# InternetMaximalism/plonky2_bn254

Hardware: NVIDIA B200
Metric: g1_scalar_mul_stark_proofs_per_sec (higher is better)
Workload: dtype u64

## Files before the change

### plonky2_bn254_b200/csrc/merkle.cuh

```cuda
#pragma once
#include "poseidon.cuh"
#include "poseidon_tc.cuh"

namespace merkle {

using poseidon::Digest;

struct LeafHashK {
  const u64* lde;
  size_t stride;
  int W, log_n;
  Digest* out;
  int natural = 0;
  PB_HD void operator()(size_t j) const {
    u64 s[12];
#pragma unroll
    for (int i = 0; i < 12; i++) s[i] = 0;
    if (W <= 4) {
      for (int c = 0; c < W; c++) s[c] = lde[(size_t)c * stride + j];
    } else {
      int c = 0;
      for (; c + 8 <= W; c += 8) {
#pragma unroll
        for (int k = 0; k < 8; k++) s[k] = lde[(size_t)(c + k) * stride + j];
        poseidon::permute(s);
      }
      if (c < W) {
        for (int k = 0; c + k < W; k++) s[k] = lde[(size_t)(c + k) * stride + j];
        poseidon::permute(s);
      }
    }
    Digest d;
#pragma unroll
    for (int i = 0; i < 4; i++) d.e[i] = s[i];
    out[natural ? j : (size_t)gl::brev32((u32)j, log_n)] = d;
  }
};

struct RowHashK {
  const u64* rows;
  int len;
  Digest* out;
  PB_HD void operator()(size_t i) const {
    u64 s[12];
#pragma unroll
    for (int k = 0; k < 12; k++) s[k] = 0;
    const u64* row = rows + i * (size_t)len;
    if (len <= 4) {
      for (int c = 0; c < len; c++) s[c] = row[c];
    } else {
      for (int c = 0; c < len; c += 8) {
        for (int k = 0; k < 8 && c + k < len; k++) s[k] = row[c + k];
        poseidon::permute(s);
      }
    }
    Digest d;
#pragma unroll
    for (int k = 0; k < 4; k++) d.e[k] = s[k];
    out[i] = d;
  }
};

struct LevelK {
  const Digest* child;
  Digest* parent;
  PB_HD void operator()(size_t i) const { parent[i] = poseidon::two_to_one(child[2 * i], child[2 * i + 1]); }
};

#if !PB_HOSTSIM
__device__ __forceinline__ void stage_rc2(u64* rc2) {
  for (int i = threadIdx.x; i < poseidon::RC2_WORDS; i += blockDim.x) rc2[i] = poseidon::RC2_DEV[i];
  __syncthreads();
}

__global__ void __launch_bounds__(poseidon::tc::CTA, poseidon::tc::CTAS_PER_SM)
    k_leaf_hash_tc(const u64* __restrict__ lde, size_t stride, int W, int log_n, Digest* __restrict__ out, size_t rows,
                   int natural) {
  extern __shared__ unsigned char tc_dyn[];
  __shared__ u64 tc_bar;
  __shared__ u32 tc_slot[2];
  poseidon::tc::Ctx ctx;
  poseidon::tc::setup(ctx, tc_dyn, &tc_bar, tc_slot);
  const size_t j = (size_t)blockIdx.x * blockDim.x + threadIdx.x;
  const bool live = j < rows;
  const u64* p = lde + (live ? j : 0);
  u64 s[12];
#pragma unroll
  for (int i = 0; i < 12; i++) s[i] = 0;
  const int chunks = (W + 7) / 8;
#pragma unroll 1
  for (int c = 0; c < chunks; c++) {
    const int len = W - 8 * c;
    const u64* q = p + (size_t)c * 8 * stride;
#pragma unroll
    for (int k = 0; k < 8; k++)
      if (k < len) s[k] = q[(size_t)k * stride];
    poseidon::tc::permute(s, ctx);
  }
  if (live) {
    Digest d;
#pragma unroll
    for (int i = 0; i < 4; i++) d.e[i] = s[i];
    out[natural ? j : (size_t)gl::brev32((u32)j, log_n)] = d;
  }
  poseidon::tc::teardown(ctx);
}

__global__ void __launch_bounds__(128, 6) k_level(const Digest* __restrict__ child, Digest* __restrict__ parent, size_t n) {
  __shared__ __align__(16) u64 rc2[poseidon::RC2_WORDS];
  stage_rc2(rc2);
  const size_t i = (size_t)blockIdx.x * blockDim.x + threadIdx.x;
  if (i >= n) return;
  u64 s[12];
  const Digest l = child[2 * i], r = child[2 * i + 1];
#pragma unroll
  for (int k = 0; k < 4; k++) {
    s[k] = l.e[k];
    s[4 + k] = r.e[k];
    s[8 + k] = 0;
  }
  poseidon::lazy::permute(s, rc2);
  Digest d;
#pragma unroll
  for (int k = 0; k < 4; k++) d.e[k] = s[k];
  parent[i] = d;
}
#endif

static inline size_t tree_digests(int log_n, int cap_height) {
  size_t total = 0;
  for (int l = log_n; l >= cap_height; l--) total += (size_t)1 << l;
  return total;
}
static inline size_t level_offset(int log_n, int lvl) {
  size_t off = 0;
  for (int l = 0; l < lvl; l++) off += (size_t)1 << (log_n - l);
  return off;
}

static inline void launch_level(const Digest* child, Digest* parent, size_t n, pbStream s) {
#if PB_HOSTSIM
  LevelK k{child, parent};
  pb_launch("merkle level", k, n, s, 128);
#else
  k_level<<<(unsigned)((n + 127) / 128), 128, 0, s>>>(child, parent, n);
  g_pb_launches++;
  pb_check_last("merkle level");
#endif
}
static inline void build_levels(Digest* digests, int log_n, int cap_height, pbStream s) {
  if (cap_height > log_n) throw Pb254Error(6, "merkle: cap_height > log2(leaves)");
  size_t off = 0;
  for (int l = 0; l < log_n - cap_height; l++) {
    size_t m = (size_t)1 << (log_n - l);
    launch_level(digests + off, digests + off + m, m / 2, s);
    off += m;
  }
}

static inline void build_from_lde(const u64* lde, size_t stride, int W, int log_n, int cap_height, Digest* digests,
                                  pbStream s) {
#if PB_HOSTSIM
  LeafHashK k{lde, stride, W, log_n, digests};
  pb_launch("leaf hash", k, (size_t)1 << log_n, s, 128);
#else
  if (W <= 4) {
    LeafHashK k{lde, stride, W, log_n, digests};
    pb_launch("leaf copy", k, (size_t)1 << log_n, s, 128);
  } else {
    const size_t n = (size_t)1 << log_n;
    k_leaf_hash_tc<<<(unsigned)((n + 127) / 128), poseidon::tc::CTA, poseidon::tc::SMEM_BYTES, s>>>(lde, stride, W, log_n,
                                                                                                  digests, n, 0);
    g_pb_launches++;
    pb_check_last("leaf hash");
  }
#endif
  build_levels(digests, log_n, cap_height, s);
}
static inline void build_from_rows(const u64* rows, int len, int log_n, int cap_height, Digest* digests, pbStream s) {
  RowHashK k{rows, len, digests};
  pb_launch("row hash", k, (size_t)1 << log_n, s, 128);
  build_levels(digests, log_n, cap_height, s);
}


static inline void hash_rows_natural(const u64* m, size_t stride, int W, size_t rows, Digest* out, pbStream s) {
#if PB_HOSTSIM
  LeafHashK k{m, stride, W, 0, out, 1};
  pb_launch("leaf hash (rows)", k, rows, s, 128);
#else
  if (W <= 4) {
    LeafHashK k{m, stride, W, 0, out, 1};
    pb_launch("leaf copy (rows)", k, rows, s, 128);
  } else {
    k_leaf_hash_tc<<<(unsigned)((rows + 127) / 128), poseidon::tc::CTA, poseidon::tc::SMEM_BYTES, s>>>(m, stride, W, 0, out,
                                                                                                     rows, 1);
    g_pb_launches++;
    pb_check_last("leaf hash (rows)");
  }
#endif
}
struct SubtreeLeavesK {
  const Digest* all;
  Digest* leaves;
  size_t first;
  int log_N;
  PB_HD void operator()(size_t q) const { leaves[q] = all[gl::brev32((u32)(first + q), log_N)]; }
};

}
```

### plonky2_bn254_b200/csrc/poseidon_tc.cuh

```cuda
#pragma once
#include "poseidon.cuh"

#if !PB_HOSTSIM
namespace poseidon {
namespace tc {

static constexpr int CTA = 128;
static constexpr int A_BYTES = 128 * 128;
static constexpr int B_BYTES = 96 * 128;
static constexpr int CTAS_PER_SM = 5;
static constexpr int SMEM_BYTES = 41 * 1024;
static_assert(A_BYTES + 2 * B_BYTES + 1024 <= SMEM_BYTES && SMEM_BYTES <= 48 * 1024, "shared-memory plan");
__host__ __device__ constexpr u32 idesc(u32 n) { return (2u << 4) | ((n >> 3) << 17) | ((128u >> 4) << 24); }

static __device__ const uint4 B_IMAGE[B_BYTES / 16] = {
#include "poseidon_constants_tcb.inc"
};
static __device__ const uint4 BF_IMAGE[B_BYTES / 16] = {
#include "poseidon_constants_tcf.inc"
};

__device__ __forceinline__ u32 smem_u32(const void* p) { return (u32)__cvta_generic_to_shared(p); }

__device__ __forceinline__ u64 smem_desc(u32 addr) {
  return (u64)((addr & 0x3FFFFu) >> 4) | ((u64)(1024u >> 4) << 32) | (1ull << 46) | (2ull << 61);
}

struct Ctx {
  unsigned char* row;
  u32 r7;
  u32 bar;
  u32 tmem0, tmem1;
  u64 adesc, bdesc, bfdesc;
  u32 parity;
};

__device__ __forceinline__ void setup(Ctx& c, unsigned char* dyn, u64* bar, u32* slot) {
  const u32 t = threadIdx.x;
  unsigned char* base = dyn + ((1024u - (smem_u32(dyn) & 1023u)) & 1023u);
  unsigned char* a = base;
  unsigned char* b = base + A_BYTES;
  unsigned char* bf = b + B_BYTES;
  for (int i = t; i < B_BYTES / 16; i += CTA) {
    reinterpret_cast<uint4*>(b)[i] = B_IMAGE[i];
    reinterpret_cast<uint4*>(bf)[i] = BF_IMAGE[i];
  }
  c.row = a + t * 128;
  c.r7 = t & 7;
  c.bar = smem_u32(bar);
  if (t == 0) {
    asm volatile("mbarrier.init.shared::cta.b64 [%0], 1;" ::"r"(c.bar));
    asm volatile("fence.mbarrier_init.release.cluster;" ::: "memory");
  }
  if (t < 32) {
    asm volatile("tcgen05.alloc.cta_group::1.sync.aligned.shared::cta.b32 [%0], 64;" ::"r"(smem_u32(slot)) : "memory");
    asm volatile("tcgen05.alloc.cta_group::1.sync.aligned.shared::cta.b32 [%0], 32;" ::"r"(smem_u32(slot + 1)) : "memory");
    asm volatile("tcgen05.relinquish_alloc_permit.cta_group::1.sync.aligned;" ::: "memory");
  }
  asm volatile("tcgen05.fence::before_thread_sync;" ::: "memory");
  __syncthreads();
  asm volatile("tcgen05.fence::after_thread_sync;" ::: "memory");
  c.tmem0 = reinterpret_cast<volatile u32*>(slot)[0];
  c.tmem1 = reinterpret_cast<volatile u32*>(slot)[1];
  c.adesc = smem_desc(smem_u32(a));
  c.bdesc = smem_desc(smem_u32(b));
  c.bfdesc = smem_desc(smem_u32(bf));
  c.parity = 0;
}

__device__ __forceinline__ void teardown(const Ctx& c) {
  asm volatile("tcgen05.fence::before_thread_sync;" ::: "memory");
  __syncthreads();
  if (threadIdx.x < 32) {
    asm volatile("tcgen05.dealloc.cta_group::1.sync.aligned.b32 %0, 64;" ::"r"(c.tmem0) : "memory");
    asm volatile("tcgen05.dealloc.cta_group::1.sync.aligned.b32 %0, 32;" ::"r"(c.tmem1) : "memory");
  }
}

template <u32 N>
__device__ __forceinline__ void mma_i8(u32 d_tmem, u64 adesc, u64 bdesc, u32 accumulate) {
  asm volatile(
      "{\n\t"
      ".reg .pred p;\n\t"
      "setp.ne.b32 p, %4, 0;\n\t"
      "tcgen05.mma.cta_group::1.kind::i8 [%0], %1, %2, %3, p;\n\t"
      "}" ::"r"(d_tmem),
      "l"(adesc), "l"(bdesc), "n"(idesc(N)), "r"(accumulate)
      : "memory");
}

#define PB_TMEM_LD32(v, addr)                                                                                       \
  asm volatile(                                                                                                     \
      "tcgen05.ld.sync.aligned.32x32b.x32.b32 {%0, %1, %2, %3, %4, %5, %6, %7, %8, %9, %10, %11, %12, %13, %14, "   \
      "%15, %16, %17, %18, %19, %20, %21, %22, %23, %24, %25, %26, %27, %28, %29, %30, %31}, [%32];"                \
      : "=r"(v[0]), "=r"(v[1]), "=r"(v[2]), "=r"(v[3]), "=r"(v[4]), "=r"(v[5]), "=r"(v[6]), "=r"(v[7]), "=r"(v[8]), \
        "=r"(v[9]), "=r"(v[10]), "=r"(v[11]), "=r"(v[12]), "=r"(v[13]), "=r"(v[14]), "=r"(v[15]), "=r"(v[16]),      \
        "=r"(v[17]), "=r"(v[18]), "=r"(v[19]), "=r"(v[20]), "=r"(v[21]), "=r"(v[22]), "=r"(v[23]), "=r"(v[24]),     \
        "=r"(v[25]), "=r"(v[26]), "=r"(v[27]), "=r"(v[28]), "=r"(v[29]), "=r"(v[30]), "=r"(v[31])                   \
      : "r"(addr)                                                                                                   \
      : "memory")

__device__ __forceinline__ u64 recombine4(u32 acc0, u32 acc1, u32 acc2, u32 acc3) {
  const u32 t1 = __byte_perm(acc1, 0, 0x1044), u1 = __byte_perm(acc1, 0, 0x4432);
  const u32 t3 = __byte_perm(acc3, 0, 0x1044), u3 = __byte_perm(acc3, 0, 0x4432);
  u32 lo, hi;
  asm("{\n\t"
      ".reg .u32 w2, c;\n\t"
      "add.cc.u32   %0, %2, %3;\n\t"
      "addc.u32     %1, %4, %5;\n\t"
      "add.cc.u32   %1, %1, %6;\n\t"
      "addc.u32     w2, %7, 0;\n\t"
      "add.cc.u32   %1, %1, w2;\n\t"
      "addc.u32     c, 0, 0;\n\t"
      "sub.cc.u32   %0, %0, w2;\n\t"
      "subc.u32     %1, %1, 0;\n\t"
      "sub.u32      c, 0, c;\n\t"
      "add.cc.u32   %0, %0, c;\n\t"
      "addc.u32     %1, %1, 0;\n\t"
      "}"
      : "=&r"(lo), "=&r"(hi)
      : "r"(acc0), "r"(t1), "r"(u1), "r"(acc2), "r"(t3), "r"(u3));
  return ((u64)hi << 32) | lo;
}

__device__ __forceinline__ u64 fold8(const u32* q) {
  return recombine4(q[0] + (q[1] << 8), q[2] + (q[3] << 8), q[4] + (q[5] << 8), q[6] + (q[7] << 8));
}


__device__ __forceinline__ u32 onehot(int p, int w) { return (p >> 2) == w ? 1u << ((p & 3) * 8) : 0u; }

__device__ __forceinline__ u32 complement4(const u64 s[12], int i0, int i1, int i2, int i3) {
  const u32 a = __byte_perm((u32)(s[i0] >> 32), (u32)(s[i1] >> 32), 0x0073);
  const u32 b = __byte_perm((u32)(s[i2] >> 32), (u32)(s[i3] >> 32), 0x0073);
  return ~__byte_perm(a, b, 0x5410);
}

__device__ __forceinline__ void product(u64 s[12], Ctx& c, u64 bdesc, uint4 x6, uint4 x7) {
#pragma unroll
  for (int ch = 0; ch < 6; ch++)
    *reinterpret_cast<uint4*>(c.row + ((ch ^ c.r7) << 4)) =
        make_uint4((u32)s[2 * ch], (u32)(s[2 * ch] >> 32), (u32)s[2 * ch + 1], (u32)(s[2 * ch + 1] >> 32));
  *reinterpret_cast<uint4*>(c.row + ((6 ^ c.r7) << 4)) = x6;
  *reinterpret_cast<uint4*>(c.row + ((7 ^ c.r7) << 4)) = x7;
  asm volatile("fence.proxy.async.shared::cta;" ::: "memory");
  asm volatile("tcgen05.fence::before_thread_sync;" ::: "memory");
  __syncthreads();
  if (threadIdx.x == 0) {
    asm volatile("tcgen05.fence::after_thread_sync;" ::: "memory");
#pragma unroll
    for (int k = 0; k < 4; k++) {
      mma_i8<64>(c.tmem0, c.adesc + 2 * k, bdesc + 2 * k, k > 0);
      mma_i8<32>(c.tmem1, c.adesc + 2 * k, bdesc + (64 * 128 >> 4) + 2 * k, k > 0);
    }
    asm volatile("tcgen05.commit.cta_group::1.mbarrier::arrive::one.shared::cluster.b64 [%0];" ::"r"(c.bar) : "memory");
  }
  {
    u32 ok;
    do {
      asm volatile(
          "{\n\t"
          ".reg .pred p;\n\t"
          "mbarrier.try_wait.parity.shared::cta.b64 p, [%1], %2;\n\t"
          "selp.u32 %0, 1, 0, p;\n\t"
          "}"
          : "=r"(ok)
          : "r"(c.bar), "r"(c.parity)
          : "memory");
    } while (!ok);
    c.parity ^= 1;
  }
  asm volatile("tcgen05.fence::after_thread_sync;" ::: "memory");
  {
    const u32 lane_off = ((threadIdx.x >> 5) * 32u) << 16;
    const u32 t0 = c.tmem0 + lane_off, t1 = c.tmem0 + lane_off + 32, t2 = c.tmem1 + lane_off;
#define PB_TC_FOLD(a, base)                                                                                   \
  _Pragma("unroll") for (int r = 0; r < 4; r++) {                                                             \
    const u32* q = a + 8 * r;                                                                                 \
    s[base + r] = fold8(q);                                                                                   \
  }
    u32 a[32], b[32];
    PB_TMEM_LD32(a, t0);
    asm volatile("tcgen05.wait::ld.sync.aligned;" ::: "memory");
    PB_TMEM_LD32(b, t1);
    PB_TC_FOLD(a, 0)
    asm volatile("tcgen05.wait::ld.sync.aligned;" ::: "memory");
    PB_TMEM_LD32(a, t2);
    PB_TC_FOLD(b, 4)
    asm volatile("tcgen05.wait::ld.sync.aligned;" ::: "memory");
    PB_TC_FOLD(a, 8)
#undef PB_TC_FOLD
  }
}

__device__ __forceinline__ void permute(u64 s[12], Ctx& c) {
#pragma unroll
  for (int i = 0; i < 12; i++) {
    const u64 k = RC_DEV[i];
    u64 t = s[i] + k;
    if (t < k) t += gl::EPS;
    s[i] = t;
  }
  constexpr int N_FUSED = N_PARTIAL / 2, N_LAYERS = 2 * HALF_FULL + N_FUSED;
#pragma unroll 1
  for (int L = 0; L < N_LAYERS; L++) {
    uint4 x6, x7;
    u64 bdesc;
    if (L < HALF_FULL || L >= HALF_FULL + N_FUSED) {
#pragma unroll 1
      for (int j = 0; j < 2; j++) {
        u64 t[6];
#pragma unroll
        for (int i = 0; i < 6; i++) t[i] = lazy::sbox(s[i]);
#pragma unroll
        for (int i = 0; i < 6; i++) {
          s[i] = s[i + 6];
          s[i + 6] = t[i];
        }
      }
      const int R = L < HALF_FULL ? L : L + N_FUSED;
      const int p = R < N_ROUNDS - 1 ? R : -1;
      x6 = make_uint4(onehot(p, 0), onehot(p, 1), onehot(p, 2), onehot(p, 3));
      x7 = make_uint4(onehot(p, 4), onehot(p, 5), onehot(p, 6), onehot(p, 7));
      bdesc = c.bdesc;
    } else {
      const int j = L - HALF_FULL, r = HALF_FULL + 2 * j;
      s[0] = lazy::sbox(s[0]);
      u32 X[6][4];
#pragma unroll
      for (int k = 0; k < 6; k++) {
        const u32 a0 = (u32)s[2 * k], a1 = (u32)(s[2 * k] >> 32), b0 = (u32)s[2 * k + 1], b1 = (u32)(s[2 * k + 1] >> 32);
        X[k][0] = __byte_perm(a0, b0, 0x5410);
        X[k][1] = __byte_perm(a0, b0, 0x7632);
        X[k][2] = __byte_perm(a1, b1, 0x5410);
        X[k][3] = __byte_perm(a1, b1, 0x7632);
      }
      const uint4 k0 = *reinterpret_cast<const uint4*>(RC2_DEV + (r + 1) * 24);
      u32 acc[4] = {k0.x, k0.y, k0.z, k0.w};
      lazy::dp_row<0, 0>(acc, X);
      const u64 t = lazy::sbox(recombine4(acc[0], acc[1], acc[2], acc[3]));
      const int p = 8 + j;
      x6 = make_uint4((u32)t, (u32)(t >> 32), onehot(p, 2), onehot(p, 3));
      x7 = make_uint4(onehot(p, 4) | (~(u32)(s[0] >> 32) & 0xFF000000u), complement4(s, 1, 2, 3, 4),
                      complement4(s, 5, 6, 7, 8), complement4(s, 9, 10, 11, 11) & 0x00FFFFFFu);
      bdesc = c.bfdesc;
    }
    product(s, c, bdesc, x6, x7);
  }
#pragma unroll
  for (int i = 0; i < 12; i++) s[i] = s[i] >= gl::P ? s[i] - gl::P : s[i];
}

}
}
#endif
```

Baseline: 5.184.

## Overlap Poseidon TC operand staging with sbox and add L2 prefetch in leaf hash

Leaf hashing moves into a grid-strided tile loop and issues L2 prefetches for the next column chunk or tile while the current permutation runs. In the fused partial rounds, the shared-memory operand rows are written early and the s[0] sbox is split out of the dot-product. Its contribution is added afterwards with dp2a, so independent work can interleave with the sbox latency. Probe template hooks are added but compile to no-ops; the grid size is unchanged, so the tile loop runs once per block.

Measured after the change: 5.199 (median of 6 runs). About the same (+0.3%).

```diff
diff --git a/plonky2_bn254_b200/csrc/merkle.cuh b/plonky2_bn254_b200/csrc/merkle.cuh
--- a/plonky2_bn254_b200/csrc/merkle.cuh
+++ b/plonky2_bn254_b200/csrc/merkle.cuh
@@ -73,6 +73,53 @@
   __syncthreads();
 }
 
+__device__ __forceinline__ void prefetch_next_chunk(const u64* lde, size_t stride, int W, size_t rows, size_t tile,
+                                                    int c) {
+  const u32 t = threadIdx.x;
+  const int col = 8 * c + (int)(t >> 3);
+  const size_t row = tile * poseidon::tc::CTA + 16 * (t & 7);
+  if (t < 64 && col < W && row < rows)
+    asm volatile("prefetch.global.L2 [%0];" ::"l"(lde + (size_t)col * stride + row));
+}
+
+template <class Probe>
+__device__ __forceinline__ void leaf_hash_tiles(poseidon::tc::Ctx& ctx, const u64* __restrict__ lde, size_t stride,
+                                                int W, int log_n, Digest* __restrict__ out, size_t rows, int natural,
+                                                Probe& pr) {
+  const size_t tiles = (rows + poseidon::tc::CTA - 1) / poseidon::tc::CTA;
+  const int chunks = (W + 7) / 8;
+#pragma unroll 1
+  for (size_t tile = blockIdx.x; tile < tiles; tile += gridDim.x) {
+    pr.tile(tile);
+    const size_t j = tile * poseidon::tc::CTA + threadIdx.x;
+    const bool live = j < rows;
+    const u64* p = lde + (live ? j : 0);
+    u64 s[12];
+#pragma unroll
+    for (int i = 0; i < 12; i++) s[i] = 0;
+#pragma unroll 1
+    for (int c = 0; c < chunks; c++) {
+      const int len = W - 8 * c;
+      const u64* q = p + (size_t)c * 8 * stride;
+#pragma unroll
+      for (int k = 0; k < 8; k++)
+        if (k < len) s[k] = q[(size_t)k * stride];
+      prefetch_next_chunk(lde, stride, W, rows, c + 1 < chunks ? tile : tile + gridDim.x, c + 1 < chunks ? c + 1 : 0);
+      poseidon::tc::permute(s, ctx, pr);
+    }
+    if (live) {
+      Digest d;
+#pragma unroll
+      for (int i = 0; i < 4; i++) d.e[i] = s[i];
+      out[natural ? j : (size_t)gl::brev32((u32)j, log_n)] = d;
+    }
+  }
+}
+
+struct NoTileProbe : poseidon::tc::NoProbe {
+  __device__ __forceinline__ void tile(size_t) {}
+};
+
 __global__ void __launch_bounds__(poseidon::tc::CTA, poseidon::tc::CTAS_PER_SM)
     k_leaf_hash_tc(const u64* __restrict__ lde, size_t stride, int W, int log_n, Digest* __restrict__ out, size_t rows,
                    int natural) {
@@ -81,29 +128,17 @@
   __shared__ u32 tc_slot[2];
   poseidon::tc::Ctx ctx;
   poseidon::tc::setup(ctx, tc_dyn, &tc_bar, tc_slot);
-  const size_t j = (size_t)blockIdx.x * blockDim.x + threadIdx.x;
-  const bool live = j < rows;
-  const u64* p = lde + (live ? j : 0);
-  u64 s[12];
-#pragma unroll
-  for (int i = 0; i < 12; i++) s[i] = 0;
-  const int chunks = (W + 7) / 8;
-#pragma unroll 1
-  for (int c = 0; c < chunks; c++) {
-    const int len = W - 8 * c;
-    const u64* q = p + (size_t)c * 8 * stride;
-#pragma unroll
-    for (int k = 0; k < 8; k++)
-      if (k < len) s[k] = q[(size_t)k * stride];
-    poseidon::tc::permute(s, ctx);
-  }
-  if (live) {
-    Digest d;
-#pragma unroll
-    for (int i = 0; i < 4; i++) d.e[i] = s[i];
-    out[natural ? j : (size_t)gl::brev32((u32)j, log_n)] = d;
-  }
+  NoTileProbe pr;
+  leaf_hash_tiles(ctx, lde, stride, W, log_n, out, rows, natural, pr);
   poseidon::tc::teardown(ctx);
+}
+
+static inline void launch_leaf_hash_tc(const u64* lde, size_t stride, int W, int log_n, Digest* out, size_t rows,
+                                       int natural, pbStream s, const char* what) {
+  const unsigned tiles = (unsigned)((rows + poseidon::tc::CTA - 1) / poseidon::tc::CTA);
+  k_leaf_hash_tc<<<tiles, poseidon::tc::CTA, poseidon::tc::SMEM_BYTES, s>>>(lde, stride, W, log_n, out, rows, natural);
+  g_pb_launches++;
+  pb_check_last(what);
 }
 
 __global__ void __launch_bounds__(128, 6) k_level(const Digest* __restrict__ child, Digest* __restrict__ parent, size_t n) {
@@ -168,11 +203,7 @@
     LeafHashK k{lde, stride, W, log_n, digests};
     pb_launch("leaf copy", k, (size_t)1 << log_n, s, 128);
   } else {
-    const size_t n = (size_t)1 << log_n;
-    k_leaf_hash_tc<<<(unsigned)((n + 127) / 128), poseidon::tc::CTA, poseidon::tc::SMEM_BYTES, s>>>(lde, stride, W, log_n,
-                                                                                                  digests, n, 0);
-    g_pb_launches++;
-    pb_check_last("leaf hash");
+    launch_leaf_hash_tc(lde, stride, W, log_n, digests, (size_t)1 << log_n, 0, s, "leaf hash");
   }
 #endif
   build_levels(digests, log_n, cap_height, s);
@@ -193,10 +224,7 @@
     LeafHashK k{m, stride, W, 0, out, 1};
     pb_launch("leaf copy (rows)", k, rows, s, 128);
   } else {
-    k_leaf_hash_tc<<<(unsigned)((rows + 127) / 128), poseidon::tc::CTA, poseidon::tc::SMEM_BYTES, s>>>(m, stride, W, 0, out,
-                                                                                                     rows, 1);
-    g_pb_launches++;
-    pb_check_last("leaf hash (rows)");
+    launch_leaf_hash_tc(m, stride, W, 0, out, rows, 1, s, "leaf hash (rows)");
   }
 #endif
 }
diff --git a/plonky2_bn254_b200/csrc/poseidon_tc.cuh b/plonky2_bn254_b200/csrc/poseidon_tc.cuh
--- a/plonky2_bn254_b200/csrc/poseidon_tc.cuh
+++ b/plonky2_bn254_b200/csrc/poseidon_tc.cuh
@@ -136,16 +136,26 @@
   return ~__byte_perm(a, b, 0x5410);
 }
 
-__device__ __forceinline__ void product(u64 s[12], Ctx& c, u64 bdesc, uint4 x6, uint4 x7) {
-#pragma unroll
-  for (int ch = 0; ch < 6; ch++)
-    *reinterpret_cast<uint4*>(c.row + ((ch ^ c.r7) << 4)) =
-        make_uint4((u32)s[2 * ch], (u32)(s[2 * ch] >> 32), (u32)s[2 * ch + 1], (u32)(s[2 * ch + 1] >> 32));
-  *reinterpret_cast<uint4*>(c.row + ((6 ^ c.r7) << 4)) = x6;
-  *reinterpret_cast<uint4*>(c.row + ((7 ^ c.r7) << 4)) = x7;
+struct NoProbe {
+  __device__ __forceinline__ void barrier(int) {}
+  __device__ __forceinline__ void issued(int) {}
+  __device__ __forceinline__ void done(int) {}
+};
+
+__device__ __forceinline__ void store_chunk(const Ctx& c, int ch, uint4 v) {
+  *reinterpret_cast<uint4*>(c.row + ((ch ^ c.r7) << 4)) = v;
+}
+__device__ __forceinline__ uint4 lane_pair(u64 a, u64 b) {
+  return make_uint4((u32)a, (u32)(a >> 32), (u32)b, (u32)(b >> 32));
+}
+
+template <class Probe>
+__device__ __forceinline__ void product(u64 s[12], Ctx& c, u64 bdesc, Probe& pr, int L) {
   asm volatile("fence.proxy.async.shared::cta;" ::: "memory");
   asm volatile("tcgen05.fence::before_thread_sync;" ::: "memory");
+  pr.barrier(L);
   __syncthreads();
+  pr.issued(L);
   if (threadIdx.x == 0) {
     asm volatile("tcgen05.fence::after_thread_sync;" ::: "memory");
 #pragma unroll
@@ -170,6 +180,7 @@
     } while (!ok);
     c.parity ^= 1;
   }
+  pr.done(L);
   asm volatile("tcgen05.fence::after_thread_sync;" ::: "memory");
   {
     const u32 lane_off = ((threadIdx.x >> 5) * 32u) << 16;
@@ -193,7 +204,8 @@
   }
 }
 
-__device__ __forceinline__ void permute(u64 s[12], Ctx& c) {
+template <class Probe>
+__device__ __forceinline__ void permute(u64 s[12], Ctx& c, Probe& pr) {
 #pragma unroll
   for (int i = 0; i < 12; i++) {
     const u64 k = RC_DEV[i];
@@ -204,7 +216,6 @@
   constexpr int N_FUSED = N_PARTIAL / 2, N_LAYERS = 2 * HALF_FULL + N_FUSED;
 #pragma unroll 1
   for (int L = 0; L < N_LAYERS; L++) {
-    uint4 x6, x7;
     u64 bdesc;
     if (L < HALF_FULL || L >= HALF_FULL + N_FUSED) {
 #pragma unroll 1
@@ -220,16 +231,20 @@
       }
       const int R = L < HALF_FULL ? L : L + N_FUSED;
       const int p = R < N_ROUNDS - 1 ? R : -1;
-      x6 = make_uint4(onehot(p, 0), onehot(p, 1), onehot(p, 2), onehot(p, 3));
-      x7 = make_uint4(onehot(p, 4), onehot(p, 5), onehot(p, 6), onehot(p, 7));
+#pragma unroll
+      for (int ch = 0; ch < 6; ch++) store_chunk(c, ch, lane_pair(s[2 * ch], s[2 * ch + 1]));
+      store_chunk(c, 6, make_uint4(onehot(p, 0), onehot(p, 1), onehot(p, 2), onehot(p, 3)));
+      store_chunk(c, 7, make_uint4(onehot(p, 4), onehot(p, 5), onehot(p, 6), onehot(p, 7)));
       bdesc = c.bdesc;
     } else {
       const int j = L - HALF_FULL, r = HALF_FULL + 2 * j;
-      s[0] = lazy::sbox(s[0]);
+#pragma unroll
+      for (int ch = 1; ch < 6; ch++) store_chunk(c, ch, lane_pair(s[2 * ch], s[2 * ch + 1]));
       u32 X[6][4];
 #pragma unroll
       for (int k = 0; k < 6; k++) {
-        const u32 a0 = (u32)s[2 * k], a1 = (u32)(s[2 * k] >> 32), b0 = (u32)s[2 * k + 1], b1 = (u32)(s[2 * k + 1] >> 32);
+        const u32 a0 = k ? (u32)s[2 * k] : 0u, a1 = k ? (u32)(s[2 * k] >> 32) : 0u;
+        const u32 b0 = (u32)s[2 * k + 1], b1 = (u32)(s[2 * k + 1] >> 32);
         X[k][0] = __byte_perm(a0, b0, 0x5410);
         X[k][1] = __byte_perm(a0, b0, 0x7632);
         X[k][2] = __byte_perm(a1, b1, 0x5410);
@@ -238,18 +253,33 @@
       const uint4 k0 = *reinterpret_cast<const uint4*>(RC2_DEV + (r + 1) * 24);
       u32 acc[4] = {k0.x, k0.y, k0.z, k0.w};
       lazy::dp_row<0, 0>(acc, X);
+      const u32 cy = complement4(s, 1, 2, 3, 4), cz = complement4(s, 5, 6, 7, 8),
+                cw = complement4(s, 9, 10, 11, 11) & 0x00FFFFFFu;
+      s[0] = lazy::sbox(s[0]);
+      store_chunk(c, 0, lane_pair(s[0], s[1]));
+      {
+        constexpr u32 m00 = lazy::Coef<0, 0>::value & 0xFFu;
+        const u32 a0 = (u32)s[0], a1 = (u32)(s[0] >> 32);
+        asm("dp2a.lo.u32.u32 %0, %1, %2, %0;" : "+r"(acc[0]) : "r"(a0), "r"(m00));
+        asm("dp2a.lo.u32.u32 %0, %1, %2, %0;" : "+r"(acc[1]) : "r"(a0), "r"(m00 << 8));
+        asm("dp2a.lo.u32.u32 %0, %1, %2, %0;" : "+r"(acc[2]) : "r"(a1), "r"(m00));
+        asm("dp2a.lo.u32.u32 %0, %1, %2, %0;" : "+r"(acc[3]) : "r"(a1), "r"(m00 << 8));
+      }
       const u64 t = lazy::sbox(recombine4(acc[0], acc[1], acc[2], acc[3]));
       const int p = 8 + j;
-      x6 = make_uint4((u32)t, (u32)(t >> 32), onehot(p, 2), onehot(p, 3));
-      x7 = make_uint4(onehot(p, 4) | (~(u32)(s[0] >> 32) & 0xFF000000u), complement4(s, 1, 2, 3, 4),
-                      complement4(s, 5, 6, 7, 8), complement4(s, 9, 10, 11, 11) & 0x00FFFFFFu);
+      store_chunk(c, 6, make_uint4((u32)t, (u32)(t >> 32), onehot(p, 2), onehot(p, 3)));
+      store_chunk(c, 7, make_uint4(onehot(p, 4) | (~(u32)(s[0] >> 32) & 0xFF000000u), cy, cz, cw));
       bdesc = c.bfdesc;
     }
-    product(s, c, bdesc, x6, x7);
+    product(s, c, bdesc, pr, L);
   }
 #pragma unroll
   for (int i = 0; i < 12; i++) s[i] = s[i] >= gl::P ? s[i] - gl::P : s[i];
 }
+__device__ __forceinline__ void permute(u64 s[12], Ctx& c) {
+  NoProbe pr;
+  permute(s, c, pr);
+}
 
 }
 }
```
